# thuml/HashGAN

Measured on AMD Instinct MI355X. Metric: queries/sec (mAP@R of Q queries vs N-code database, Hamming ranking), higher is better.
Workload: dtype fp4 (E2M1 0/+-1) x fp4 -> f32 exact distances; u32 xor+popcount elsewhere; f64 AP; 1 GPU; C2: Q=10000 N=1000000 b=64 R=5000 C=10, planted codes; parallelism=1 GPU

## Files before the change

### hashgan_amd/csrc/hg_rank_lean.hpp

```cpp
#pragma once
#include "hg_rank_cnt.hpp"

namespace hg {

#ifndef HG_RL_INFLIGHT
#define HG_RL_INFLIGHT 4
#endif
constexpr int RL_NPT = 4;
constexpr int RL_MAX_PIECES = 256 * RL_NPT;

struct RankLeanLds { int cnt, off, tot, misc, bm, pref, rec, total; };
__host__ __device__ inline RankLeanLds rank_lean_layout(int NB, i64 RW, int S, int rec_bytes, int nbc) {
    RankLeanLds l;
    const int RC_MAXB = rank_cnt_maxb(NB);
    const int NBall = NB < 128 ? NB : 128;
    const int NBc = nbc > 0 && nbc < NBall ? nbc : NBall;
    l.cnt = 0;
    int cb = (NBc + 1) * 256;
    if (cb < AP_LDS_BYTES + 8) cb = AP_LDS_BYTES + 8;
    l.off = (cb + 15) & ~15;
    l.tot = l.off + (RC_MAXB + 1) * 512;
    l.misc = l.tot + ((NB + 3) & ~3) * 4;
    l.bm = l.misc + 64;
    l.pref = (l.bm + (int)(2 * RW) * 4 + 16 + 15) & ~15;
    l.rec = (l.pref + (S + 4) * 4 + 15) & ~15;
    l.total = l.rec + rec_bytes;
    return l;
}

template <int CTRL, int ROWS> __device__ __forceinline__ u32 rl_dpp_add(const u32 v) {
    return v + (u32)__builtin_amdgcn_update_dpp(0, (int)v, CTRL, ROWS, 0xF, false);
}
__device__ __forceinline__ u32 rl_scan(u32 v) {
    v = rl_dpp_add<0x111, 0xF>(v);
    v = rl_dpp_add<0x112, 0xF>(v);
    v = rl_dpp_add<0x114, 0xF>(v);
    v = rl_dpp_add<0x118, 0xF>(v);
    v = rl_dpp_add<0x142, 0xA>(v);
    v = rl_dpp_add<0x143, 0xC>(v);
    return v;
}

static __global__ __launch_bounds__(256) __attribute__((amdgpu_waves_per_eu(HG_RANK_WAVES, HG_RANK_WAVES)))
void k_rank_lean(const u8* __restrict__ cand8, const RankLdsArgs a, u32* __restrict__ mbits32, const Geo g) {
    extern __shared__ __attribute__((aligned(16))) u8 rlds[];
    const int q = logical_block(g.Q);
    if (q < 0) return;
    const int tid = threadIdx.x;
    const int lane = tid & 63;
    const int wave = __builtin_amdgcn_readfirstlane(tid >> 6);
    const int NB = g.NB, S = g.S;
    const int NBall = NB < 128 ? NB : 128;
    const int NBc = a.nbc > 0 && a.nbc < NBall ? a.nbc : NBall;
    const int RC_MAXB = rank_cnt_maxb(NB);
    const int bmw = (int)(2 * a.RW);
    constexpr int nthr = 256;
    const RankLeanLds L = rank_lean_layout(NB, a.RW, S, a.lds_recs, a.nbc);
    u32* cnt32 = (u32*)(rlds + L.cnt);
    u32* off32 = (u32*)(rlds + L.off);
    u32* tot = (u32*)(rlds + L.tot);
    u32* misc = (u32*)(rlds + L.misc);
    u32* bm = (u32*)(rlds + L.bm);
    u32* pref = (u32*)(rlds + L.pref);
    u8* rec8 = rlds + L.rec;
    u32* __restrict__ grow = mbits32 + (i64)q * 2 * a.RW;

#ifdef HG_RANK_PROFILE
    const unsigned long long tk0 = __builtin_amdgcn_s_memtime();
    int tkn = 0;
#define HG_TKL() do { if (tid == 0 && q < 4096) a.hwq[(i64)q * 16 + tkn] = (u32)(__builtin_amdgcn_s_memtime() - tk0); ++tkn; } while (0)
#else
#define HG_TKL() do {} while (0)
#endif

    const u32 failed = a.fail[q];
    const int T = a.cut ? a.cut[q] : NB - 1;
    const u32 c_s = tid < S ? a.sl_cnt[(i64)tid * g.Qpad + q] : 0u;
    const int PPS = (int)(a.cap >> 4);
    const int PSP = a.spec_pieces;
    const int TP = S * PSP;
    const u32 inv = (65536u + (u32)PSP - 1u) / (u32)PSP;
    const uint4* __restrict__ row16 = (const uint4*)(cand8 + (i64)q * a.crow);
    uint4 spec[RL_NPT];
#pragma unroll
    for (int k = 0; k < RL_NPT; ++k) {
        const u32 p = (u32)(tid + nthr * k);
        const u32 s = (p * inv) >> 16, ps = p - s * (u32)PSP;
        spec[k] = p < (u32)TP ? row16[s * (u32)PPS + ps] : uint4{0u, 0u, 0u, 0u};
    }
    for (int i = tid * 16; i < L.pref; i += nthr * 16) *(uint4*)(rlds + i) = uint4{0u, 0u, 0u, 0u};

    if (tid == 0) a.big[q] = 0u;
    if (failed) {
        if (tid == 0) {
            if (a.mode == 3) atomicOr(&a.hown[(i64)NB * g.Qpad], 1u);
            else { atomicExch(a.err, 1); a.qbad[q] = 1u; }
        }
        if (a.mode == 3) for (int d = tid; d < NB; d += nthr) a.hown[(i64)d * g.Qpad + q] = 0u;
        return;
    }
    const int wlo = a.cut ? (T - (NBc - 1) > 0 ? T - (NBc - 1) : 0) : 0;
    const u32 pad = (u32)(wlo + NBc);

    const u32 pc = (c_s + 15u) >> 4;
    const u32 incl = rl_scan(pc);
    if (lane == 63) pref[S + wave] = incl;
    __syncthreads();
    u32 wbase = 0, n16 = 0;
#pragma unroll
    for (int w = 0; w < 4; ++w) {
        const u32 v = pref[S + w];
        wbase += w < wave ? v : 0u;
        n16 += v;
    }
    if (tid < S) pref[tid] = (wbase + incl - pc) | (c_s << 16);
    if (T > 126 || n16 * 16u > (u32)a.lds_recs || n16 > (u32)RL_MAX_PIECES) {
        if (tid == 0) { a.big[q] = 1u; if (a.nleft) atomicAdd(a.nleft, 1u); }
        return;
    }
    __syncthreads();
    HG_TKL();

    const u32 padw = pad * 0x01010101u;
    auto put_piece = [&](const uint4 v, const int valid, const u32 dst) {
        u32 w[4] = {v.x, v.y, v.z, v.w};
        if (valid < 16) {
#pragma unroll
            for (int i = 0; i < 4; ++i) {
                const int nb = valid - 4 * i;
                const u32 keep = nb >= 4 ? 0xFFFFFFFFu : nb <= 0 ? 0u : (1u << (8 * nb)) - 1u;
                w[i] = (w[i] & keep) | (padw & ~keep);
            }
        }
        *(uint4*)(rec8 + 16u * dst) = uint4{w[0], w[1], w[2], w[3]};
    };
#pragma unroll
    for (int k = 0; k < RL_NPT; ++k) {
        const u32 p = (u32)(tid + nthr * k);
        if (p < (u32)TP) {
            const u32 s = (p * inv) >> 16, ps = p - s * (u32)PSP;
            const u32 e = pref[s];
            const int valid = (int)(e >> 16) - (int)(16u * ps);
            if (valid > 0) put_piece(spec[k], valid, (e & 0xFFFFu) + ps);
        }
    }
    if (pc > (u32)PSP) {
        const u32 first = wbase + incl - pc;
        for (u32 ps = (u32)PSP; ps < pc; ++ps) put_piece(row16[(u32)tid * (u32)PPS + ps], (int)c_s - (int)(16u * ps), first + ps);
    }
    __syncthreads();
    HG_TKL();

    const int PPT = (int)((n16 + nthr - 1) / nthr);
    const u32 p0 = (u32)tid * (u32)PPT;
    uint4 ch[RL_NPT];
#pragma unroll
    for (int k = 0; k < RL_NPT; ++k)
        if (k < PPT && p0 + k < n16) ch[k] = *(const uint4*)(rec8 + 16u * (p0 + k));
        else ch[k] = uint4{0u, 0u, 0u, 0u};
    {
        const u32 one = 1u << (8 * (tid & 3));
        u8* cbase = (u8*)cnt32 + (tid >> 2) * 4;
        u32 mx = 0;
#pragma unroll
        for (int k = 0; k < RL_NPT; ++k) {
            if (k < PPT && p0 + k < n16) {
                const u32 w[4] = {ch[k].x, ch[k].y, ch[k].z, ch[k].w};
#pragma unroll
                for (int i = 0; i < 16; ++i) {
                    const u32 d = (w[i >> 2] >> (8 * (i & 3))) & 0x7Fu;
                    const u32 rel = d - (u32)wlo;
                    mx = rel > mx ? rel : mx;
                    const u32 row = rel < (u32)NBc ? rel : (u32)NBc;
                    atomicAdd((u32*)(cbase + row * 256u), one);
                }
            }
        }
        if (mx > (u32)NBc) misc[7] = 1u;
    }
    __syncthreads();
    HG_TKL();
    if (misc[7]) { if (tid == 0) { a.big[q] = 1u; if (a.nleft) atomicAdd(a.nleft, 1u); } return; }
    {
        const int d = tid >> 2, j = tid & 3;
        u32 sm = 0;
        if (d < NBc) {
            const uint4* c4 = (const uint4*)(cnt32 + d * 64 + j * 16);
#pragma unroll
            for (int k = 0; k < 4; ++k) {
                const uint4 v = c4[k];
                sm += __builtin_amdgcn_sad_u8(v.x, 0u, 0u) + __builtin_amdgcn_sad_u8(v.y, 0u, 0u) + __builtin_amdgcn_sad_u8(v.z, 0u, 0u) +
                      __builtin_amdgcn_sad_u8(v.w, 0u, 0u);
            }
        }
        sm += (u32)__builtin_amdgcn_update_dpp(0, (int)sm, 0xB1, 0xF, 0xF, false);
        sm += (u32)__builtin_amdgcn_update_dpp(0, (int)sm, 0x4E, 0xF, 0xF, false);
        if (d < NBc && j == 0 && wlo + d < NB) tot[wlo + d] = sm;
    }
    __syncthreads();
    HG_TKL();
    if (a.mode == 3) for (int d = tid; d < NB; d += nthr) a.hown[(i64)d * g.Qpad + q] = tot[d];

    const bool has = lane < NBc && wlo + lane < NB;
    const u32 ctot = has ? tot[wlo + lane] : 0u;
    const u32 cinc = rl_scan(ctot);
    const u32 cstart = cinc - ctot;
    u64 want = (u64)g.R;
    if (a.mode == 3) {
        const u32 have = (u32)__builtin_amdgcn_readlane((int)cinc, 63);
        if ((u64)have < want) want = have;
    }
    const u64 present = __ballot(ctot != 0u);
    const u64 reached = want > 0 ? __ballot(has && (u64)cinc >= want) : 0ull;
    const int t = reached ? wlo + (int)__builtin_ctzll(reached) : -1;
    if (tid == 0 && a.mode == 0) {
        if (t < 0) atomicExch(a.err, 1);
        a.qbad[q] = t < 0 ? 1u : 0u;
    }
    if (t < 0) {
        if (a.mode == 3) for (int w = tid; w < bmw; w += nthr) grow[w] = 0u;
        return;
    }
    const int dmin = wlo + (int)__builtin_ctzll(present);
    const int nbk = t - dmin + 1;
    if (nbk > RC_MAXB) {
        if (tid == 0) { a.big[q] = 1u; if (a.nleft) atomicAdd(a.nleft, 1u); }
        return;
    }
    for (int k = wave; k < nbk; k += 4) {
        const int row = dmin + k - wlo;
        const u32 x = cnt32[row * 64 + lane];
        const u32 sm = __builtin_amdgcn_sad_u8(x, 0u, 0u);
        const u32 inc = rl_scan(sm);
        const u32 o0 = (u32)__builtin_amdgcn_readlane((int)cstart, row) + inc - sm;
        const u32 o1 = o0 + (x & 0xFFu), o2 = o1 + ((x >> 8) & 0xFFu), o3 = o2 + ((x >> 16) & 0xFFu);
        *(uint2*)(off32 + k * 128 + 2 * lane) = uint2{o0 | (o1 << 16), o2 | (o3 << 16)};
    }
    if (tid < 128) off32[RC_MAXB * 128 + tid] = (u32)want * 0x00010001u;
    __syncthreads();
    HG_TKL();

    {
        const u32 sh = 16u * (u32)(tid & 1);
        const u32 one = 1u << sh;
        u8* obase = (u8*)off32 + (tid >> 1) * 4;
        const u32 wantu = (u32)want;
#pragma unroll
        for (int k = 0; k < RL_NPT; ++k) {
            if (k < PPT && p0 + k < n16) {
                const u32 w[4] = {ch[k].x, ch[k].y, ch[k].z, ch[k].w};
                constexpr int GR = HG_RL_INFLIGHT;
#pragma unroll
                for (int i0 = 0; i0 < 16; i0 += GR) {
                    u32 r[GR];
#pragma unroll
                    for (int e = 0; e < GR; ++e) {
                        const int d = (int)((w[(i0 + e) >> 2] >> (8 * ((i0 + e) & 3))) & 0x7Fu);
                        const int kk = d > t ? RC_MAXB : d - dmin;
                        r[e] = atomicAdd((u32*)(obase + kk * 512), one);
                    }
#pragma unroll
                    for (int e = 0; e < GR; ++e) {
                        const u32 pos = (r[e] >> sh) & 0xFFFFu;
                        if (((w[(i0 + e) >> 2] >> (8 * ((i0 + e) & 3) + 7)) & 1u) && pos < wantu) atomicOr(&bm[pos >> 5], 1u << (pos & 31));
                    }
                }
            }
        }
    }
    __syncthreads();
    HG_TKL();
    for (int w = tid; w < bmw; w += nthr) grow[w] = bm[w];
    HG_TKL();
    if (a.ap_shapes) {
        const u64* bm64 = (const u64*)bm;
        if (a.ap_recip) ap_eval2<nthr>([&](const i64 w) { return bm64[w]; }, a.RW, g.R, a.ap_shapes, a.ap_recip, ap_lds_at(rlds + L.cnt), tid, a.ap + q, a.rel + q);
        else ap_eval<nthr>([&](const i64 w) { return bm64[w]; }, a.RW, g.R, a.ap_shapes, a.ap_recip, ap_lds_at(rlds + L.cnt), tid, a.ap + q, a.rel + q);
        HG_TKL();
    }
}

}
```

Before: 12.64 million queries/s.

## Remap LDS counter lanes by wave and use SWAR byte math in lean ranking

Changes the LDS histogram and offset counter layout so that each byte or halfword slot is selected by wave index and the word address by lane, instead of interleaving by thread id. The distance bias and the overflow check are now done four bytes at a time with SWAR arithmetic. The offset scan is split into packed lo/hi halfword scans, and offset rows past nbk are filled with the 'want' sentinel. The scatter pass clamps with a single unsigned compare against RC_MAXB. The aim is fewer ALU ops per code and fewer LDS atomic bank conflicts. The cost is a more intricate packed-scan layout that must stay consistent across the count, offset and scatter stages.

New measurement: 12.74 million queries/s (median of 6 runs). Within noise of the previous version (+0.8%).

```diff
diff --git a/hashgan_amd/csrc/hg_rank_lean.hpp b/hashgan_amd/csrc/hg_rank_lean.hpp
--- a/hashgan_amd/csrc/hg_rank_lean.hpp
+++ b/hashgan_amd/csrc/hg_rank_lean.hpp
@@ -159,24 +159,28 @@
         if (k < PPT && p0 + k < n16) ch[k] = *(const uint4*)(rec8 + 16u * (p0 + k));
         else ch[k] = uint4{0u, 0u, 0u, 0u};
     {
-        const u32 one = 1u << (8 * (tid & 3));
-        u8* cbase = (u8*)cnt32 + (tid >> 2) * 4;
-        u32 mx = 0;
+        const u32 one = 1u << (8 * wave);
+        u8* cbase = (u8*)cnt32 + lane * 4;
+        const u32 wlow = (u32)wlo * 0x01010101u, topw = (u32)(0x7F - NBc) * 0x01010101u;
+        u32 out = 0;
 #pragma unroll
         for (int k = 0; k < RL_NPT; ++k) {
             if (k < PPT && p0 + k < n16) {
                 const u32 w[4] = {ch[k].x, ch[k].y, ch[k].z, ch[k].w};
 #pragma unroll
-                for (int i = 0; i < 16; ++i) {
-                    const u32 d = (w[i >> 2] >> (8 * (i & 3))) & 0x7Fu;
-                    const u32 rel = d - (u32)wlo;
-                    mx = rel > mx ? rel : mx;
-                    const u32 row = rel < (u32)NBc ? rel : (u32)NBc;
-                    atomicAdd((u32*)(cbase + row * 256u), one);
+                for (int j = 0; j < 4; ++j) {
+                    const u32 x = (w[j] & 0x7F7F7F7Fu) - wlow;
+                    out |= (x | (x + topw)) & 0x80808080u;
+#pragma unroll
+                    for (int i = 0; i < 4; ++i) {
+                        const u32 rel = (x >> (8 * i)) & 0xFFu;
+                        const u32 row = rel < (u32)NBc ? rel : (u32)NBc;
+                        atomicAdd((u32*)(cbase + row * 256u), one);
+                    }
                 }
             }
         }
-        if (mx > (u32)NBc) misc[7] = 1u;
+        if (out) misc[7] = 1u;
     }
     __syncthreads();
     HG_TKL();
@@ -230,33 +234,42 @@
     for (int k = wave; k < nbk; k += 4) {
         const int row = dmin + k - wlo;
         const u32 x = cnt32[row * 64 + lane];
-        const u32 sm = __builtin_amdgcn_sad_u8(x, 0u, 0u);
-        const u32 inc = rl_scan(sm);
-        const u32 o0 = (u32)__builtin_amdgcn_readlane((int)cstart, row) + inc - sm;
-        const u32 o1 = o0 + (x & 0xFFu), o2 = o1 + ((x >> 8) & 0xFFu), o3 = o2 + ((x >> 16) & 0xFFu);
-        *(uint2*)(off32 + k * 128 + 2 * lane) = uint2{o0 | (o1 << 16), o2 | (o3 << 16)};
-    }
-    if (tid < 128) off32[RC_MAXB * 128 + tid] = (u32)want * 0x00010001u;
-    __syncthreads();
-    HG_TKL();
-
-    {
-        const u32 sh = 16u * (u32)(tid & 1);
+        const u32 lo = x & 0x00FF00FFu, hi = (x >> 8) & 0x00FF00FFu;
+        const u32 ilo = rl_scan(lo), ihi = rl_scan(hi);
+        const u32 tlo = (u32)__builtin_amdgcn_readlane((int)ilo, 63), thi = (u32)__builtin_amdgcn_readlane((int)ihi, 63);
+        const u32 elo = ilo - lo, ehi = ihi - hi;
+        const u32 s0 = (u32)__builtin_amdgcn_readlane((int)cstart, row);
+        const u32 s1 = s0 + (tlo & 0xFFFFu), s2 = s1 + (thi & 0xFFFFu), s3 = s2 + (tlo >> 16);
+        const u32 o0 = s0 + (elo & 0xFFFFu), o1 = s1 + (ehi & 0xFFFFu), o2 = s2 + (elo >> 16), o3 = s3 + (ehi >> 16);
+        off32[k * 128 + lane] = o0 | (o2 << 16);
+        off32[k * 128 + 64 + lane] = o1 | (o3 << 16);
+    }
+    {
+        const u32 wp = (u32)want * 0x00010001u;
+        for (int i = nbk * 32 + tid; i < (RC_MAXB + 1) * 32; i += nthr) ((uint4*)off32)[i] = uint4{wp, wp, wp, wp};
+    }
+    __syncthreads();
+    HG_TKL();
+
+    {
+        const u32 sh = 16u * (u32)(wave >> 1);
         const u32 one = 1u << sh;
-        u8* obase = (u8*)off32 + (tid >> 1) * 4;
+        u8* obase = (u8*)off32 + (lane + 64 * (wave & 1)) * 4;
+        const u32 dminw = (u32)dmin * 0x01010101u;
         const u32 wantu = (u32)want;
 #pragma unroll
         for (int k = 0; k < RL_NPT; ++k) {
             if (k < PPT && p0 + k < n16) {
                 const u32 w[4] = {ch[k].x, ch[k].y, ch[k].z, ch[k].w};
+                const u32 x[4] = {(w[0] & 0x7F7F7F7Fu) - dminw, (w[1] & 0x7F7F7F7Fu) - dminw, (w[2] & 0x7F7F7F7Fu) - dminw, (w[3] & 0x7F7F7F7Fu) - dminw};
                 constexpr int GR = HG_RL_INFLIGHT;
 #pragma unroll
                 for (int i0 = 0; i0 < 16; i0 += GR) {
                     u32 r[GR];
 #pragma unroll
                     for (int e = 0; e < GR; ++e) {
-                        const int d = (int)((w[(i0 + e) >> 2] >> (8 * ((i0 + e) & 3))) & 0x7Fu);
-                        const int kk = d > t ? RC_MAXB : d - dmin;
+                        const u32 rel = (x[(i0 + e) >> 2] >> (8 * ((i0 + e) & 3))) & 0xFFu;
+                        const u32 kk = rel < (u32)RC_MAXB ? rel : (u32)RC_MAXB;
                         r[e] = atomicAdd((u32*)(obase + kk * 512), one);
                     }
 #pragma unroll
```
